# zhai-lw/L3AC

Measured on AMD Instinct MI355X. Metric: audio samples/sec encode+decode, 1kbps@16kHz, batch 256; indices bit-exact, higher is better.
Workload: dtype f32

## Files before the change

include/l3ac_hip.h:

```cpp
#ifndef L3AC_HIP_H
#define L3AC_HIP_H

#include <stddef.h>
#include <stdint.h>

#ifdef __cplusplus
extern "C" {
#endif

#define L3AC_ABI_VERSION 5
#define L3AC_MAX_STAGES 8
#define L3AC_MAX_LEVELS 8

enum {
    L3AC_OK = 0,
    L3AC_EINVAL = -1,
    L3AC_EWEIGHT = -2,
    L3AC_EHIP = -3,
    L3AC_ENOMEM = -4,
    L3AC_ECOOP = -5,
};

typedef struct l3ac_config {
    int32_t abi_version;
// ... 168 lines not shown
               double fmin, double fmax, int32_t window, int32_t hop, double threshold, double* f0, int32_t* voiced, double* aperiodicity,
               double* cmnd, int32_t* frames, void* scratch, int64_t scratch_bytes, void* stream);
int l3ac_pitch_metrics(const double* f0_ref, const int32_t* voiced_ref, const double* f0_est, const int32_t* voiced_est, int32_t batch,
                       int64_t max_frames, const int32_t* frames, double* out, int32_t* counts, void* stream);

typedef struct l3ac_pack_stream_desc {
    int32_t slot;
    int32_t held;
    int32_t take;
    int32_t count;
    int32_t keep;
} l3ac_pack_stream_desc;
typedef struct l3ac_unpack_stream_desc {
    int32_t slot;
    int32_t held;
    int32_t take;
    int32_t count;
    int32_t keep;
} l3ac_unpack_stream_desc;
int64_t l3ac_packed_bytes(int64_t n_tok, int32_t bits);
int l3ac_pack_stream(const uint32_t* state_in, uint32_t* state_out, int32_t streams, const int32_t* fresh, int64_t fresh_tokens,
                     int64_t fresh_stride, int32_t bits, const l3ac_pack_stream_desc* desc, int32_t count, uint8_t* out, int64_t out_bytes,
                     int64_t out_stride, void* stream);
int l3ac_unpack_stream(const uint32_t* state_in, uint32_t* state_out, int32_t streams, const uint8_t* fresh, int64_t fresh_bytes,
                       int64_t fresh_stride, int32_t bits, const l3ac_unpack_stream_desc* desc, int32_t count, int32_t* out, int64_t out_tokens,
                       int64_t out_stride, void* stream);

int l3ac_op_first_block(l3ac_ctx* ctx, const float* audio, int32_t batch, int32_t samples, float* y, void* stream);
int l3ac_op_first_block_at(l3ac_ctx* ctx, const float* audio, int32_t batch, int32_t samples, int64_t audio_stride, int32_t frames,
                           float* y, void* stream);
int l3ac_op_conv_unit(l3ac_ctx* ctx, const char* block, const float* x, int32_t batch, int32_t frames, float* y,
                      void* stream);
int l3ac_op_down_layer(l3ac_ctx* ctx, const char* block, const float* x, int32_t batch, int32_t frames, float* y,
                       void* stream);
int l3ac_op_conv_k3(l3ac_ctx* ctx, const char* block, const float* x, int32_t batch, int32_t frames, float* y,
                    void* stream);
int l3ac_op_enhance(l3ac_ctx* ctx, const char* block, const float* x, int32_t batch, int32_t frames, float* y,
                    void* stream);
int l3ac_op_up_layer(l3ac_ctx* ctx, const char* block, const float* x, int32_t batch, int32_t frames, float* y,
                     void* stream);
int l3ac_op_enhance_up(l3ac_ctx* ctx, const char* enhance_block, const char* up_block, const float* x, int32_t batch,
                       int32_t frames, float* y, void* stream);
int l3ac_op_last_block(l3ac_ctx* ctx, const float* x, int32_t batch, int32_t frames, float* audio, void* stream);
int l3ac_op_legacy_unit(l3ac_ctx* ctx, int32_t unit, const float* x, int32_t batch, int32_t frames, float* y, void* stream);
int l3ac_op_head(l3ac_ctx* ctx, const float* x, int32_t batch, int32_t frames, float* audio, void* stream);
int l3ac_op_local_trans(l3ac_ctx* ctx, const char* block, const float* x, int32_t batch, int32_t frames, float* y,
                        void* stream);
int l3ac_op_encoder(l3ac_ctx* ctx, const float* audio, int32_t batch, int32_t samples, float* feature, void* stream);
int l3ac_op_en_encoder(l3ac_ctx* ctx, const float* feature, int32_t batch, int32_t frames, float* tokens, void* stream);
int l3ac_op_en_decoder(l3ac_ctx* ctx, const float* tokens, int32_t batch, int32_t n_tok, float* feature, void* stream);
int l3ac_op_decoder(l3ac_ctx* ctx, const float* feature, int32_t batch, int32_t frames, float* audio, void* stream);

int l3ac_op_snake(const float* x, float* y, int64_t rows, int32_t c, const float* alpha, int32_t mode, void* stream);
int l3ac_ctx_set_head_pretanh(l3ac_ctx* ctx, int32_t enable);

typedef struct l3ac_profile_entry {
    char name[64];
    int32_t launches;
    int32_t reserved;
    double ms_total;
    double flops;
    double bytes;
} l3ac_profile_entry;
int l3ac_profile_begin(void);
int l3ac_profile_end(l3ac_profile_entry* out, int32_t cap, int32_t* n_out);

int l3ac_gemm_f32(const float* a, int64_t lda, const float* w, const float* bias, float* c, int64_t ldc,
                  int64_t m, int32_t n, int32_t k, void* stream);

void l3ac_split3_host(const float* x, int64_t n, uint16_t* planes);
int l3ac_ctx_set_gemm_split(l3ac_ctx* ctx, int32_t enable);
int l3ac_ctx_set_option(l3ac_ctx* ctx, const char* name, int32_t value);
int l3ac_ctx_get_option(const l3ac_ctx* ctx, const char* name, int32_t* out);
int32_t l3ac_ctx_get_gemm_split(const l3ac_ctx* ctx);
int64_t l3ac_gemm_split_image_bytes(int32_t n, int32_t k);
int l3ac_gemm_split_image(const float* w, int32_t n, int32_t k, void* image, void* stream);
int l3ac_gemm_split_f32(const float* a, int64_t lda, const void* image, const float* bias, float* c, int64_t ldc,
                        int64_t m, int32_t n, int32_t k, void* stream);
int l3ac_gemm_split_f32_at(const float* a, int64_t lda, const void* image, const float* bias, float* c, int64_t ldc,
                           int64_t m, int32_t n, int32_t k, int32_t w256, void* stream);

#ifdef __cplusplus
}
#endif
#endif
```

l3ac_amd/_capi.py:

```python
from __future__ import annotations

import ctypes as C
from pathlib import Path

import os

LIB_PATH = Path(os.environ.get("L3AC_LIB_PATH") or Path(__file__).resolve().parent / "libl3ac_hip.so")
ABI_VERSION = 5
MAX_STAGES = 8
MAX_LEVELS = 8


class L3acError(RuntimeError):
    pass


class Config(C.Structure):
    _fields_ = [
        ("abi_version", C.c_int32),
        ("feature_dim", C.c_int32),
        ("n_enc", C.c_int32),
        ("enc_dims", C.c_int32 * MAX_STAGES),
        ("enc_depths", C.c_int32 * MAX_STAGES),
        ("compress_rates", C.c_int32 * MAX_STAGES),
# ... 28 lines not shown
    _fields_ = [("slot", C.c_int32), ("held", C.c_int32), ("take", C.c_int32), ("count", C.c_int32), ("keep", C.c_int32)]


class UnpackStreamDesc(C.Structure):
    _fields_ = [("slot", C.c_int32), ("held", C.c_int32), ("take", C.c_int32), ("count", C.c_int32), ("keep", C.c_int32)]


class Tensor(C.Structure):
    _fields_ = [("name", C.c_char_p), ("data", C.c_void_p), ("numel", C.c_int64)]


_P, _I32, _I64 = C.c_void_p, C.c_int32, C.c_int64
SIGNATURES = {
    "l3ac_last_error": (C.c_char_p, []),
    "l3ac_abi_version": (C.c_int, []),
    "l3ac_create": (C.c_int, [C.POINTER(Config), C.POINTER(Tensor), _I32, _I32, C.POINTER(_P)]),
    "l3ac_destroy": (None, [_P]),
    "l3ac_reserve": (C.c_int, [_P, _I32, _I32]),
    "l3ac_workspace_bytes": (_I64, [_P]),
    "l3ac_grn_min_norm": (C.c_int, [_P, _I32, C.POINTER(C.c_float)]),
    "l3ac_bad_index_count": (C.c_int, [_P, _I32, C.POINTER(_I64)]),
    "l3ac_coop_timeout_count": (C.c_int, [_P, _I32, C.POINTER(_I64)]),
    "l3ac_coop_timeout_pending": (C.c_int, [_P, C.POINTER(_I64)]),
    "l3ac_coop_claimed_cus": (_I32, [_I32]),
    "l3ac_hop_length": (_I32, [_P]),
    "l3ac_encode": (C.c_int, [_P, _P, _I32, _I32, _I64, _P, _P, _P, _P]),
    "l3ac_decode": (C.c_int, [_P, _P, _P, _I32, _I32, _P, _P]),
    "l3ac_encode_ragged": (C.c_int, [_P, _P, _I32, _I32, _I64, C.POINTER(_I32), _P, _P, _P, _P]),
    "l3ac_decode_ragged": (C.c_int, [_P, _P, _P, _I32, _I32, C.POINTER(_I32), _P, _P]),
    "l3ac_fsq_forward": (C.c_int, [_P, _I64, _I32, C.POINTER(_I32), _I32, _P, _P, _P, _P, _P, _P, _P, _P, _P]),
    "l3ac_fsq_quantize_act": (C.c_int, [_P, _I64, _I32, C.POINTER(_I32), _I32, _P, _P, _P, _P, _P, _P]),
    "l3ac_fsq_decode": (C.c_int, [_P, _I64, _I32, C.POINTER(_I32), _I32, _P, _P, _P, _P]),
    "l3ac_fsq_copy_ceiling": (C.c_int, [_P, _I64, _P, _P, _P, _P]),
    "l3ac_fsq_copy_ceiling_at": (C.c_int, [_P, _I64, _P, _P, _P, _I32, _P]),
    "l3ac_vq_argmin_scratch_bytes": (_I64, [_I64, _I32, _I32]),
    "l3ac_vq_argmin": (C.c_int, [_P, _I64, _P, _I32, _I32, _P, _P, _I64, _I32, _P]),
    "l3ac_op_first_block": (C.c_int, [_P, _P, _I32, _I32, _P, _P]),
    "l3ac_op_first_block_at": (C.c_int, [_P, _P, _I32, _I32, _I64, _I32, _P, _P]),
    "l3ac_op_conv_unit": (C.c_int, [_P, C.c_char_p, _P, _I32, _I32, _P, _P]),
    "l3ac_op_down_layer": (C.c_int, [_P, C.c_char_p, _P, _I32, _I32, _P, _P]),
    "l3ac_op_conv_k3": (C.c_int, [_P, C.c_char_p, _P, _I32, _I32, _P, _P]),
    "l3ac_op_enhance": (C.c_int, [_P, C.c_char_p, _P, _I32, _I32, _P, _P]),
    "l3ac_op_up_layer": (C.c_int, [_P, C.c_char_p, _P, _I32, _I32, _P, _P]),
    "l3ac_op_enhance_up": (C.c_int, [_P, C.c_char_p, C.c_char_p, _P, _I32, _I32, _P, _P]),
    "l3ac_op_last_block": (C.c_int, [_P, _P, _I32, _I32, _P, _P]),
    "l3ac_op_legacy_unit": (C.c_int, [_P, _I32, _P, _I32, _I32, _P, _P]),
    "l3ac_op_head": (C.c_int, [_P, _P, _I32, _I32, _P, _P]),
    "l3ac_op_local_trans": (C.c_int, [_P, C.c_char_p, _P, _I32, _I32, _P, _P]),
    "l3ac_op_encoder": (C.c_int, [_P, _P, _I32, _I32, _P, _P]),
    "l3ac_op_en_encoder": (C.c_int, [_P, _P, _I32, _I32, _P, _P]),
    "l3ac_op_en_decoder": (C.c_int, [_P, _P, _I32, _I32, _P, _P]),
    "l3ac_op_decoder": (C.c_int, [_P, _P, _I32, _I32, _P, _P]),
    "l3ac_op_snake": (C.c_int, [_P, _P, _I64, _I32, _P, _I32, _P]),
    "l3ac_ctx_set_head_pretanh": (C.c_int, [_P, _I32]),
    "l3ac_gemm_f32": (C.c_int, [_P, _I64, _P, _P, _P, _I64, _I64, _I32, _I32, _P]),
    "l3ac_split3_host": (None, [_P, _I64, _P]),
    "l3ac_ctx_set_gemm_split": (C.c_int, [_P, _I32]),
    "l3ac_ctx_set_option": (C.c_int, [_P, C.c_char_p, _I32]),
    "l3ac_ctx_get_option": (C.c_int, [_P, C.c_char_p, C.POINTER(_I32)]),
    "l3ac_ctx_get_gemm_split": (_I32, [_P]),
    "l3ac_gemm_split_image_bytes": (_I64, [_I32, _I32]),
    "l3ac_gemm_split_image": (C.c_int, [_P, _I32, _I32, _P, _P]),
    "l3ac_gemm_split_f32": (C.c_int, [_P, _I64, _P, _P, _P, _I64, _I64, _I32, _I32, _P]),
    "l3ac_gemm_split_f32_at": (C.c_int, [_P, _I64, _P, _P, _P, _I64, _I64, _I32, _I32, _I32, _P]),
    "l3ac_pack_indices": (C.c_int, [_P, _I32, _I32, _I32, _P, _I32, _P]),
    "l3ac_unpack_indices": (C.c_int, [_P, _I32, _I32, _I32, _I32, _P, _P]),
    "l3ac_resample_length": (_I64, [_I32, _I32, _I64]),
    "l3ac_resample_bank": (_I64, [_I32, _I32, _P, _I64]),
    "l3ac_resample": (C.c_int, [_P, _I32, _I64, _I64, _I32, _I32, _P, _P, _I64, _P]),
    "l3ac_chunk_plan": (_I64, [C.POINTER(_I64), _I32, _I64, _I64, _I32, C.POINTER(ChunkDesc), _I64]),
    "l3ac_chunk_cut": (C.c_int, [_P, _I32, _I64, _I32, C.POINTER(ChunkDesc), _I32, _P, _I32, _I64, _P]),
    "l3ac_chunk_merge": (C.c_int, [_P, _I32, _I64, _I32, C.POINTER(ChunkDesc), _I32, _P, _I32, _I64, _I64, _P]),
    "l3ac_stream_gather": (C.c_int, [_P, _I32, _I64, _P, _I64, _I64, _I32, C.POINTER(StreamDesc), _I32, _P, _I32, _I64, _P]),
    "l3ac_stream_carry": (C.c_int, [_P, _I32, _I64, _I32, C.POINTER(StreamDesc), _I32, _P, _I32, _I64, _P]),
    "l3ac_stream_append": (C.c_int, [_P, _I64, _I64, _I32, C.POINTER(StreamDesc), _I32, _P, _I32, _I64, _P]),
    "l3ac_stream_emit": (C.c_int, [_P, _I32, _I64, _I32, C.POINTER(StreamDesc), _I32, _P, _I32, _I64, _I64, _P]),
    "l3ac_resample_stream_state": (_I64, [_I32, _I32]),
    "l3ac_resample_stream": (C.c_int, [_P, _P, _I32, _I64, _P, _I64, _I64, _I32, _I32, _P, C.POINTER(ResampleStreamDesc), _I32, _P, _I64, _I64, _P]),
    "l3ac_packed_bytes": (_I64, [_I64, _I32]),
    "l3ac_pack_stream": (C.c_int, [_P, _P, _I32, _P, _I64, _I64, _I32, C.POINTER(PackStreamDesc), _I32, _P, _I64, _I64, _P]),
    "l3ac_unpack_stream": (C.c_int, [_P, _P, _I32, _P, _I64, _I64, _I32, C.POINTER(UnpackStreamDesc), _I32, _P, _I64, _I64, _P]),
    "l3ac_stft_frames": (_I64, [_I64, _I32]),
    "l3ac_stft_basis": (_I64, [_I32, _P, _I64]),
    "l3ac_mel_weights": (_I64, [_I32, _I32, _I32, _P, _I64]),
    "l3ac_mel_scratch_bytes": (_I64, [_I32, _I64, _I32, _I32, _I32]),
    "l3ac_stft": (C.c_int, [_P, _I32, _I64, _I64, C.POINTER(_I32), _I32, _I32, _P, _P, _P, _I64, _P]),
    "l3ac_log_mel": (C.c_int, [_P, _I32, _I64, _I64, C.POINTER(_I32), _I32, _I32, _P, _P, _I32, _P, _P, _I64, _P]),
    "l3ac_mel_distance": (C.c_int, [_P, _I64, _P, _I64, _I32, _I64, C.POINTER(_I32), _I32, _I32, _I32, _P, _P, _P, _P, _I64, _P]),
    "l3ac_signal_metrics": (C.c_int, [_P, _I64, _P, _I64, _I32, _I64, C.POINTER(_I32), _P, _P, _I64, _P]),
    "l3ac_stoi_frames": (_I64, [_I64]),
    "l3ac_stoi_basis": (_I64, [_P, _I64]),
    "l3ac_stoi_window": (_I64, [_P, _I64]),
    "l3ac_stoi_bands": (C.c_int, [C.POINTER(_I32)]),
    "l3ac_stoi_scratch_bytes": (_I64, [_I32, _I64]),
    "l3ac_stoi": (C.c_int, [_P, _I64, _P, _I64, _I32, _I64, C.POINTER(_I32), _P, _P, _P, _P, _P, _I64, _P]),
    "l3ac_loudness_coeffs": (_I64, [_I32, _P, _I64]),
    "l3ac_loudness_blocks": (_I64, [_I64, _I32]),
    "l3ac_loudness_scratch_bytes": (_I64, [_I32, _I64, _I32]),
    "l3ac_loudness": (C.c_int, [_P, _I64, _I32, _I64, C.POINTER(_I32), _I32, _P, _P, _P, _P, _I64, _P]),
    "l3ac_loudness_gain": (C.c_int, [_P, _I32, C.c_double, C.c_double, _P, _P]),
    "l3ac_apply_gain": (C.c_int, [_P, _I64, _P, _I64, _I32, _I64, C.POINTER(_I32), _P, _I64, _P]),
    "l3ac_pitch_lags": (C.c_int, [_I32, C.c_double, C.c_double, _I32, _I32, C.POINTER(_I32)]),
    "l3ac_pitch_frames": (_I64, [_I64, _I32, C.c_double, C.c_double, _I32, _I32]),
    "l3ac_pitch_scratch_bytes": (_I64, [_I32, _I64, _I32, C.c_double, C.c_double, _I32, _I32]),
    "l3ac_pitch": (C.c_int, [_P, _I64, _I32, _I64, C.POINTER(_I32), _I32, C.c_double, C.c_double, _I32, _I32, C.c_double, _P, _P, _P, _P, _P, _P,
                             _I64, _P]),
# ... 164 lines not shown
```

l3ac_amd/build.py:

```python
from __future__ import annotations

import os
import shutil
import subprocess
import sys
from concurrent.futures import ThreadPoolExecutor
from pathlib import Path

PKG = Path(__file__).resolve().parent
REPO = PKG.parent
CSRC = PKG / "csrc"
_TAG = os.environ.get("L3AC_BUILD_TAG", "")
OBJ_DIR = CSRC / (f"build_{_TAG}" if _TAG else "build")
LIB_PATH = PKG / (f"libl3ac_hip_{_TAG}.so" if _TAG else "libl3ac_hip.so")
ARCH = "gfx950"

SOURCES = [
    "capi.hip",
    "network.hip",
    "kernels/gemm_f32.hip",
    "kernels/gemm_split.hip",
    "kernels/gemm_split_w256.hip",
    "kernels/rows.hip",
    "kernels/first_block.hip",
# ... 79 lines not shown
        return []
    return extra


def _flag_stamp(hipcc: str, flags) -> str:
    import hashlib
    ver = subprocess.run([hipcc, "--version"], capture_output=True, text=True).stdout
    per_file = "\n".join(f"{k}: {' '.join(_per_file_flags(hipcc, k))}" for k in sorted(PER_FILE_FLAGS))
    return hashlib.sha256(("\n".join(flags) + "\n" + per_file + "\n" + ver).encode()).hexdigest()


def build_library(force: bool = False, verbose: bool = False) -> Path:
    OBJ_DIR.mkdir(parents=True, exist_ok=True)
    hipcc = _hipcc()
    flags = [*os.environ.get("L3AC_EXTRA_HIPCC_FLAGS", "").split(), "-O3", "-std=c++17", f"--offload-arch={ARCH}", "-fPIC", "-Wall", "-Wno-unused-function",
             f"-I{REPO / 'include'}", f"-I{CSRC}"]
    hdr_time = _newest_header()
    stamp_file = OBJ_DIR / "flags.sha256"
    stamp = _flag_stamp(hipcc, flags)
    if not stamp_file.exists() or stamp_file.read_text().strip() != stamp:
        force = True
    jobs = []
    objs = []
    for src in SOURCES:
        s = CSRC / src
        o = OBJ_DIR / (src.replace("/", "_") + ".o")
        d = o.with_suffix(".d")
        objs.append(o)
        stale = force or not o.exists()
        if not stale:
            newest = max(s.stat().st_mtime, _depfile_newest(d) if d.exists() else hdr_time)
            stale = o.stat().st_mtime < newest
        if stale:
            jobs.append([hipcc, *flags, *_per_file_flags(hipcc, src), "-MD", "-MF", str(d), "-c", str(s), "-o", str(o)])

    def run(cmd):
        if verbose:
            print(" ".join(cmd), flush=True)
        r = subprocess.run(cmd, capture_output=True, text=True)
        if r.returncode != 0:
            raise RuntimeError(f"hipcc failed: {' '.join(cmd)}\n{r.stdout}\n{r.stderr}")
        if verbose and r.stderr.strip():
            print(r.stderr, file=sys.stderr)

    with ThreadPoolExecutor(max_workers=min(4, os.cpu_count() or 1)) as pool:
        list(pool.map(run, jobs))
    stamp_file.write_text(stamp + "\n")
    linked = bool(jobs) or not LIB_PATH.exists()
    if linked:
        run([hipcc, "-shared", "-fPIC", f"--offload-arch={ARCH}", "-o", str(LIB_PATH), *map(str, objs)])
    global last_build_report
    last_build_report = {"objects": len(objs), "compiled": len(jobs), "reused": len(objs) - len(jobs), "linked": linked,
                         "forced": bool(force)}
    return LIB_PATH


last_build_report = None


if __name__ == "__main__":
    path = build_library(force="--force" in sys.argv, verbose=True)
    r = last_build_report
    print(f"built {path} ({path.stat().st_size / 1e6:.1f} MB): {r['compiled']} of {r['objects']} objects compiled, {r['reused']} reused")
```

l3ac_amd/csrc/capi.hip:

```cpp
#include <algorithm>
#include <cmath>
#include <cstdarg>
#include <cstdlib>
#include <cstring>
#include <new>
#include <string>
#include <vector>

#include "network.hpp"
#include "kernels/split_bf16.hpp"

static thread_local std::string g_last_error;

void l3ac_set_error(const char* fmt, ...) {
    char buf[1024];
    va_list ap;
    va_start(ap, fmt);
    vsnprintf(buf, sizeof(buf), fmt, ap);
    va_end(ap);
    g_last_error = buf;
}

int l3ac_device_cu_count() {
    static std::atomic<int> cus[L3AC_MAX_DEVICES] = {};
    const int slot = l3ac_device_slot();
    int v = slot >= 0 ? cus[slot].load(std::memory_order_relaxed) : 0;
    if (v <= 0) {
        int dev = 0;
        if (hipGetDevice(&dev) != hipSuccess || hipDeviceGetAttribute(&v, hipDeviceAttributeMultiprocessorCount, dev) != hipSuccess || v <= 0) v = 256;
        if (slot >= 0) cus[slot].store(v, std::memory_order_relaxed);
    }
    return v;
}

static thread_local Profiler* g_profiler = nullptr;
Profiler* l3ac_current_profiler() { return g_profiler; }
void l3ac_set_current_profiler(Profiler* p) { g_profiler = p; }

namespace {

struct DeviceGuard {
    int prev = -1;
    bool ok = true;
    explicit DeviceGuard(int dev) {
        if (hipGetDevice(&prev) != hipSuccess) prev = -1;
        if (prev != dev && hipSetDevice(dev) != hipSuccess) ok = false;
        if (prev == dev) prev = -1;
    }
    ~DeviceGuard() {
        if (prev >= 0) (void)hipSetDevice(prev);
    }
};

#define L3AC_ENTER(ctx)                                     \
    L3AC_REQUIRE((ctx) != nullptr, "null context");         \
    DeviceGuard guard_((ctx)->device);                      \
    L3AC_REQUIRE(guard_.ok, "cannot select device %d", (ctx)->device)
// ... 836 lines not shown
        out[slot].launches += 1;
        out[slot].ms_total += ms;
        out[slot].flops += r.flops;
        out[slot].bytes += r.bytes;
    }
    if (p->failed && rc == L3AC_OK) {
        l3ac_set_error("profile: event creation failed");
        rc = L3AC_EHIP;
    }
    delete p;
    if (n_out) *n_out = n;
    return rc;
}

int l3ac_gemm_f32(const float* a, int64_t lda, const float* w, const float* bias, float* c, int64_t ldc, int64_t m,
                  int32_t n, int32_t k, void* stream) {
    GemmArgs g{};
    g.a = a; g.lda = lda; g.w = w; g.ldw = k; g.c = c; g.ldc = ldc; g.m = m; g.n = n; g.k = k; g.bias = bias; g.epi = EPI_BIAS;
    return launch_gemm((hipStream_t)stream, g);
}

void l3ac_split3_host(const float* x, int64_t n, uint16_t* planes) {
    for (int64_t i = 0; i < n; ++i) {
        uint16_t pl[3];
        split3_host(x[i], pl);
        planes[i] = pl[0];
        planes[n + i] = pl[1];
        planes[2 * n + i] = pl[2];
    }
}

int l3ac_ctx_set_head_pretanh(l3ac_ctx* ctx, int32_t enable) { return l3ac_ctx_set_option(ctx, "head_pretanh", enable); }

int l3ac_op_snake(const float* x, float* y, int64_t rows, int32_t c, const float* alpha, int32_t mode, void* stream) {
    L3AC_REQUIRE(x && y && alpha && rows >= 0 && c > 0 && c % 4 == 0 && c <= 4096 && mode >= 0 && mode <= 4, "op_snake: bad arguments");
    hipStream_t s = (hipStream_t)stream;
    float* inv = nullptr;
    std::vector<float> ha((size_t)c), hi((size_t)c);
    L3AC_HIP_CHECK(hipMemcpyAsync(ha.data(), alpha, (size_t)c * sizeof(float), hipMemcpyDeviceToHost, s));
    L3AC_HIP_CHECK(hipStreamSynchronize(s));
    for (int i = 0; i < c; ++i) hi[i] = 1.0f / (ha[i] + 1e-8f);
    L3AC_HIP_CHECK(hipMalloc((void**)&inv, (size_t)c * sizeof(float)));
    int rc = L3AC_OK;
    if (hipMemcpyAsync(inv, hi.data(), (size_t)c * sizeof(float), hipMemcpyHostToDevice, s) != hipSuccess) {
        l3ac_set_error("op_snake: upload failed");
        rc = L3AC_EHIP;
    }
    if (rc == L3AC_OK) rc = launch_snake(s, x, y, rows, c, alpha, inv, mode);
    (void)hipStreamSynchronize(s);
    (void)hipFree(inv);
    return rc;
}

int l3ac_ctx_set_option(l3ac_ctx* ctx, const char* name, int32_t value) {
    L3AC_REQUIRE(ctx != nullptr && name != nullptr, "set_option: null argument");
    if (std::strcmp(name, "coop_release_claim") == 0) {
        trans_coop_release(ctx->coop);
        return L3AC_OK;
    }
    if (std::strcmp(name, "coop_test_fault") == 0) {
        ctx->coop.fault_part = value - 1;
        return L3AC_OK;
    }
    const Option* o = find_option(name);
    return o ? set_checked(ctx, *o, value, "set_option") : unknown_option("set_option", name);
}

int l3ac_ctx_get_option(const l3ac_ctx* ctx, const char* name, int32_t* out) {
    L3AC_REQUIRE(ctx != nullptr && name != nullptr && out != nullptr, "get_option: null argument");
    const Option* o = find_option(name);
    if (!o) return unknown_option("get_option", name);
    *out = o->field(const_cast<l3ac_ctx&>(*ctx));
    return L3AC_OK;
}

int l3ac_ctx_set_gemm_split(l3ac_ctx* ctx, int32_t enable) { return l3ac_ctx_set_option(ctx, "gemm_split", enable); }
int32_t l3ac_ctx_get_gemm_split(const l3ac_ctx* ctx) { int32_t v = 0; return l3ac_ctx_get_option(ctx, "gemm_split", &v) == L3AC_OK ? v : 0; }

int64_t l3ac_gemm_split_image_bytes(int32_t n, int32_t k) {
    return (n > 0 && k > 0 && gemm_split_eligible(n, k)) ? gemm_split_image_bytes(n, k) : 0;
}

int l3ac_gemm_split_image(const float* w, int32_t n, int32_t k, void* image, void* stream) {
    L3AC_REQUIRE(gemm_split_eligible(n, k), "split image: shape n=%d k=%d is not eligible (n >= 192, k >= 32, k %% 8 == 0)", n, k);
    return launch_gemm_split_image((hipStream_t)stream, w, k, n, k, (unsigned char*)image);
}

int l3ac_gemm_split_f32_at(const float* a, int64_t lda, const void* image, const float* bias, float* c, int64_t ldc, int64_t m,
                           int32_t n, int32_t k, int32_t w256, void* stream) {
    L3AC_REQUIRE(w256 >= 0 && w256 <= 2, "split gemm: w256 = %d, not 0, 1 or 2", w256);
    GemmArgs g{};
    g.a = a; g.lda = lda; g.w_img = (const unsigned char*)image; g.c = c; g.ldc = ldc; g.m = m; g.n = n; g.k = k; g.bias = bias;
    g.epi = EPI_BIAS; g.w256 = w256;
    return launch_gemm_split((hipStream_t)stream, g);
}
int l3ac_gemm_split_f32(const float* a, int64_t lda, const void* image, const float* bias, float* c, int64_t ldc, int64_t m,
                        int32_t n, int32_t k, void* stream) {
    const Option& o = *find_option("gemm_w256");
    return l3ac_gemm_split_f32_at(a, lda, image, bias, c, ldc, m, n, k, checked_value(o, initial_value(o)), stream);
}

}
```

l3ac_amd/csrc/kernels/gemm_split_common.hpp:

```cpp
#pragma once

#include <type_traits>

#include "../kernels.hpp"
#include "device_math.hpp"
#include "gemm_epilogue.hpp"
#include "split_bf16.hpp"

namespace {

constexpr int BM = 128, BN = 128, BK = 32, THREADS = 256;
constexpr int W_PLANE = BN * 64;
constexpr int W_TILE = 3 * W_PLANE;
constexpr int W_LOADS = W_TILE / (16 * THREADS);
static_assert(W_TILE == L3AC_SPLIT_TILE_BYTES, "image geometry");

__host__ __device__ __forceinline__ int tile_off(int row, int chunk) { return row * 64 + ((chunk ^ ((0 - (row >> 2)) & 3)) << 4); }

typedef float f32x4a __attribute__((ext_vector_type(4)));
__device__ __forceinline__ void c_store(float* p, float v) { __builtin_nontemporal_store(v, p); }

template <int RG, int NT = 8>
__device__ __forceinline__ void gemm_epilogue16(const GemmArgs& p, f32x4a (&acc)[RG][NT], int64_t m0, int n0, int wave, int lane) {
    const int c32 = lane & 31, hi = lane >> 5;
// ... 54 lines not shown
                        f32x2 hv;
                        hv.x = half ? up[i] : lo[i];
                        hv.y = half ? up[i + 1] : lo[i + 1];
                        const f32x2 sv = snake_act2(hv + bi, al, ia);
                        const f32x2 o = p.epi == EPI_SNAKE_GRN ? __builtin_elementwise_fma(ga, sv, be) + sv : sv;
                        const int64_t m = mw + 16 * h + 4 * half + i;
                        if (m < p.m) c_store(p.c + m * p.ldc + n, o.x);
                        if (m + 1 < p.m) c_store(p.c + (m + 1) * p.ldc + n, o.y);
                    }
                continue;
            }
#pragma unroll
            for (int half = 0; half < 2; ++half)
#pragma unroll
                for (int i = 0; i < 4; ++i) {
                    const int64_t m = mw + 16 * h + 4 * half + i;
                    if (m >= p.m) continue;
                    float v = (half ? up[i] : lo[i]) + bias;
                    if (p.epi == EPI_BIAS_RES) v = p.res[m * p.ldres + n] + v;
                    c_store(p.c + m * p.ldc + n, v);
                }
        }
    }
}

template <int RG, int NQ, class AccAt>
__device__ __forceinline__ void epilogue_rows(const GemmArgs& p, AccAt&& acc_at, int64_t m0, int n0, int wave, int lane, float* tb) {
    {
    const int er = lane >> 4, eq = lane & 15, ln = lane & 15, lg = lane >> 4;
    const int64_t mw = m0 + 16 * RG * wave;
#pragma unroll
    for (int sq = 0; sq < NQ; ++sq) {
        const int col = n0 + 64 * sq + 4 * eq;
        const bool col_ok = col < p.n;
        const int colc = col_ok ? col : 0;
        typedef float f4 __attribute__((ext_vector_type(4)));
        const f4 bias = p.bias ? *reinterpret_cast<const f4*>(p.bias + colc) : f4{0.f, 0.f, 0.f, 0.f};
        f4 alpha = {0.f, 0.f, 0.f, 0.f}, inv_alpha = alpha, gamma = alpha, beta = alpha;
        if (p.epi == EPI_SNAKE || p.epi == EPI_SNAKE_GRN) {
            alpha = *reinterpret_cast<const f4*>(p.alpha + colc);
            inv_alpha = *reinterpret_cast<const f4*>(p.inv_alpha + colc);
        }
        if (p.epi == EPI_SNAKE_GRN) {
            gamma = *reinterpret_cast<const f4*>(p.gamma + colc);
            beta = *reinterpret_cast<const f4*>(p.beta + colc);
        }
#pragma unroll
        for (int h = 0; h < RG; ++h) {
            float* const sb = tb + 1024 * ((sq * RG + h) & 1);
#pragma unroll
            for (int tt = 0; tt < 4; ++tt)
#pragma unroll
                for (int i = 0; i < 4; ++i) sb[(4 * lg + i) * 64 + 16 * tt + ln] = acc_at(sq, h, tt)[i];
#pragma unroll
            for (int jr = 0; jr < 4; ++jr) {
                const int64_t m = mw + 16 * h + er + 4 * jr;
                f4 v = *reinterpret_cast<const f4*>(sb + (er + 4 * jr) * 64 + 4 * eq);
                if (m >= p.m || !col_ok) continue;
                v = v + bias;
                if (p.epi == EPI_SNAKE || p.epi == EPI_SNAKE_GRN) {
                    const f32x2 s0 = snake_act2(f32x2{v.x, v.y}, f32x2{alpha.x, alpha.y}, f32x2{inv_alpha.x, inv_alpha.y});
                    const f32x2 s1 = snake_act2(f32x2{v.z, v.w}, f32x2{alpha.z, alpha.w}, f32x2{inv_alpha.z, inv_alpha.w});
                    if (p.epi == EPI_SNAKE_GRN) {
                        const f32x2 o0 = __builtin_elementwise_fma(f32x2{gamma.x, gamma.y}, s0, f32x2{beta.x, beta.y}) + s0;
                        const f32x2 o1 = __builtin_elementwise_fma(f32x2{gamma.z, gamma.w}, s1, f32x2{beta.z, beta.w}) + s1;
                        v = f4{o0.x, o0.y, o1.x, o1.y};
                    } else {
                        v = f4{s0.x, s0.y, s1.x, s1.y};
                    }
                } else if (p.epi == EPI_BIAS_RES) {
                    v = *reinterpret_cast<const f4*>(p.res + m * p.ldres + col) + v;
                }
                __builtin_nontemporal_store(v, reinterpret_cast<f4*>(p.c + m * p.ldc + col));
            }
        }
    }
}
}

template <int N, class F, int I = 0>
__device__ __forceinline__ void tail_for(F&& f) {
    if constexpr (I < N) {
        f(std::integral_constant<int, I>{});
        tail_for<N, F, I + 1>(static_cast<F&&>(f));
    }
}

}
```

l3ac_amd/csrc/kernels/rows.hip:

```cpp
#include "../kernels.hpp"
#include "device_math.hpp"
#include "lane_sums.hpp"

namespace {

constexpr int THREADS = 256;
constexpr int MAX_CH = 2;

__device__ __forceinline__ float group_sum(float v, int lpr, int pos) {
    if ((lpr & (lpr - 1)) == 0) return lanes_sum(v, lpr);
    for (int d = 1; d < lpr; d <<= 1) {
        const float o = __shfl_down(v, d, 64);
        v += pos + d < lpr ? o : 0.f;
    }
    return __shfl(v, (int)(threadIdx.x & 63) - pos, 64);
}

__device__ __forceinline__ float4 f4_fma(float4 a, float4 b, float4 c) {
    return make_float4(fmaf(a.x, b.x, c.x), fmaf(a.y, b.y, c.y), fmaf(a.z, b.z, c.z), fmaf(a.w, b.w, c.w));
}

template <int SRC, int NORM, class IDX, int LPR, int NCH>
__global__ __launch_bounds__(THREADS) void row_kernel(const RowArgs p, const int lpr_rt) {
    const int lpr = LPR ? LPR : lpr_rt;
    const int gpw = 64 / lpr;
    const int lane = threadIdx.x & 63;
    const int grp = lane / lpr;
    const int j = lane - grp * lpr;
    const IDX rows = (IDX)(p.batch * p.frames_out);
    const IDX frames_out = (IDX)p.frames_out, frames_in = (IDX)p.frames_in, cc = (IDX)p.c;
    const int nchunk = p.c >> 2;
    const IDX wave_id = (IDX)blockIdx.x * (THREADS / 64) + (threadIdx.x >> 6);
    const IDX row_step = (IDX)gridDim.x * (THREADS / 64) * gpw;
    for (IDX row = grp < gpw ? wave_id * gpw + grp : rows; row < rows; row += row_step) {
    const bool row_ok = true;
    const IDX b = row / frames_out;
    const IDX t = row - b * frames_out;

    float4 v[NCH];
    bool ok[NCH];
#pragma unroll
    for (int i = 0; i < NCH; ++i) {
        const int chunk = j + i * lpr;
        ok[i] = row_ok && chunk < nchunk;
        v[i] = make_float4(0.f, 0.f, 0.f, 0.f);
        if (!ok[i]) continue;
        const int c0 = chunk << 2;
        if (SRC == SRC_PLAIN) {
            v[i] = *reinterpret_cast<const float4*>(p.x + (size_t)((b * frames_in + t) * cc + (IDX)c0));
        } else if (SRC == SRC_DWCONV7) {
            float4 acc = *reinterpret_cast<const float4*>(p.dw_b + c0);
#pragma unroll
            for (int tap = 0; tap < 7; ++tap) {
                const int64_t ts = (int64_t)t + tap - 3;
                if (ts >= 0 && ts < p.frames_in) {
                    const float4 xv = *reinterpret_cast<const float4*>(p.x + (size_t)((b * frames_in + (IDX)ts) * cc + (IDX)c0));
                    const float4 wv = *reinterpret_cast<const float4*>(p.dw_w + tap * p.c + c0);
                    acc = f4_fma(xv, wv, acc);
                }
            }
// ... 26 lines not shown
            const float4 xv = *reinterpret_cast<const float4*>(p.x + (size_t)((b * frames_in + t) * cc + (IDX)c0));
            const float4 gb = *reinterpret_cast<const float4*>(p.gate_b + c0);
            const float xs[4] = {xv.x, xv.y, xv.z, xv.w};
            const float gbs[4] = {gb.x, gb.y, gb.z, gb.w};
            float o[4];
#pragma unroll
            for (int e = 0; e < 4; ++e) {
                const float4 gw = *reinterpret_cast<const float4*>(p.gate_w + (int64_t)(c0 + e) * 4);
                const float g = gbs[e] + gw.x * y0 + gw.y * y1 + gw.z * y2 + gw.w * y3;
                o[e] = xs[e] + g * xs[e];
            }
            v[i] = make_float4(o[0], o[1], o[2], o[3]);
        }
    }

    if (NORM != NORM_NONE) {
        float s = 0.f;
#pragma unroll
        for (int i = 0; i < NCH; ++i) s += (v[i].x + v[i].y) + (v[i].z + v[i].w);
        const float mean = group_sum(s, lpr, j) / (float)p.c;
        float q = 0.f;
#pragma unroll
        for (int i = 0; i < NCH; ++i) {
            if (ok[i]) {
                const float dx = v[i].x - mean, dy = v[i].y - mean, dz = v[i].z - mean, dw = v[i].w - mean;
                q += (dx * dx + dy * dy) + (dz * dz + dw * dw);
            }
        }
        const float var = group_sum(q, lpr, j) / (float)p.c;
        const float rstd = 1.0f / sqrtf(var + p.eps);
#pragma unroll
        for (int i = 0; i < NCH; ++i) {
            if (!ok[i]) continue;
            const int c0 = (j + i * lpr) << 2;
            const float4 w = *reinterpret_cast<const float4*>(p.nw + c0);
            const float4 bb = *reinterpret_cast<const float4*>(p.nb + c0);
            if (NORM == NORM_LN) {
                v[i] = make_float4((v[i].x - mean) * rstd * w.x + bb.x, (v[i].y - mean) * rstd * w.y + bb.y,
                                   (v[i].z - mean) * rstd * w.z + bb.z, (v[i].w - mean) * rstd * w.w + bb.w);
            } else {
                v[i] = make_float4(w.x * ((v[i].x - mean) * rstd) + bb.x, w.y * ((v[i].y - mean) * rstd) + bb.y,
                                   w.z * ((v[i].z - mean) * rstd) + bb.z, w.w * ((v[i].w - mean) * rstd) + bb.w);
            }
        }
    }
#pragma unroll
    for (int i = 0; i < NCH; ++i) {
        if (ok[i]) *reinterpret_cast<float4*>(p.y + (size_t)(row * cc + (IDX)((j + i * lpr) << 2))) = v[i];
    }
    }
}


template <int CH>
__global__ __launch_bounds__(THREADS) void dwconv_ln_kernel(const RowArgs p, const int lpr, const int DW_SEG) {
    const int groups_per_block = THREADS / lpr;
    const int64_t seg_per_clip = (p.frames_out + DW_SEG - 1) / DW_SEG;
    const int64_t seg = (int64_t)blockIdx.x * groups_per_block + threadIdx.x / lpr;
    const int j = threadIdx.x % lpr;
    const bool seg_ok = seg < p.batch * seg_per_clip;
    const int64_t sg = seg_ok ? seg : 0;
    const int64_t b = sg / seg_per_clip;
    const int t0 = (int)(sg % seg_per_clip) * DW_SEG;
    const int frames = (int)p.frames_in;
    const int nchunk = p.c >> 2;
    const float* clip = p.x + b * p.frames_in * p.c;
    float* dst = p.y + b * p.frames_in * p.c;

    bool ok[CH];
    int c0[CH];
    float4 wt[7][CH], bias[CH], lw[CH], lb[CH], win[7][CH];
#pragma unroll
    for (int i = 0; i < CH; ++i) {
        const int chunk = j + i * lpr;
        ok[i] = seg_ok && chunk < nchunk;
        c0[i] = (ok[i] ? chunk : 0) << 2;
        bias[i] = *reinterpret_cast<const float4*>(p.dw_b + c0[i]);
        lw[i] = *reinterpret_cast<const float4*>(p.nw + c0[i]);
        lb[i] = *reinterpret_cast<const float4*>(p.nb + c0[i]);
#pragma unroll
        for (int tap = 0; tap < 7; ++tap) wt[tap][i] = *reinterpret_cast<const float4*>(p.dw_w + tap * p.c + c0[i]);
    }
    auto load_row = [&](int t, int i) -> float4 {
        if (ok[i] && t >= 0 && t < frames) return *reinterpret_cast<const float4*>(clip + (int64_t)t * p.c + c0[i]);
        return make_float4(0.f, 0.f, 0.f, 0.f);
    };
#pragma unroll
    for (int d = -3; d <= 2; ++d)
#pragma unroll
        for (int i = 0; i < CH; ++i) win[(d + 7) % 7][i] = load_row(t0 + d, i);

    for (int base = 0; base < DW_SEG; base += 7) {
#pragma unroll
        for (int u = 0; u < 7; ++u) {
            const int t = t0 + base + u;
#pragma unroll
            for (int i = 0; i < CH; ++i) win[(u + 3) % 7][i] = load_row(t + 3, i);
            float4 v[CH];
            float s = 0.f;
#pragma unroll
            for (int i = 0; i < CH; ++i) {
                float4 acc = bias[i];
#pragma unroll
                for (int tap = 0; tap < 7; ++tap) acc = f4_fma(win[(u + tap + 4) % 7][i], wt[tap][i], acc);
                v[i] = ok[i] ? acc : make_float4(0.f, 0.f, 0.f, 0.f);
                s += (v[i].x + v[i].y) + (v[i].z + v[i].w);
            }
            const float mean = group_sum(s, lpr, j) / (float)p.c;
            float q = 0.f;
#pragma unroll
            for (int i = 0; i < CH; ++i) {
                if (ok[i]) {
                    const float dx = v[i].x - mean, dy = v[i].y - mean, dz = v[i].z - mean, dw = v[i].w - mean;
                    q += (dx * dx + dy * dy) + (dz * dz + dw * dw);
                }
            }
            const float rstd = 1.0f / sqrtf(group_sum(q, lpr, j) / (float)p.c + p.eps);
            if (t < frames) {
#pragma unroll
                for (int i = 0; i < CH; ++i) {
                    if (!ok[i]) continue;
                    *reinterpret_cast<float4*>(dst + (int64_t)t * p.c + c0[i]) =
                        make_float4((v[i].x - mean) * rstd * lw[i].x + lb[i].x, (v[i].y - mean) * rstd * lw[i].y + lb[i].y,
                                    (v[i].z - mean) * rstd * lw[i].z + lb[i].z, (v[i].w - mean) * rstd * lw[i].w + lb[i].w);
                }
            }
        }
    }
}

int launch_dwconv_ln(hipStream_t s, const RowArgs& r, int lpr) {
    const int64_t rows_per_wave_group = (r.batch * r.frames_out * lpr / 64) / (256 * 4 * 6);
    int DW_SEG = (int)(rows_per_wave_group / 7) * 7;
    DW_SEG = DW_SEG < 7 ? 7 : (DW_SEG > 56 ? 56 : DW_SEG);
    const int64_t segs = r.batch * ((r.frames_out + DW_SEG - 1) / DW_SEG);
    const int64_t blocks = ceil_div64(segs, THREADS / lpr);
    if (blocks <= 0) return L3AC_OK;
    L3AC_REQUIRE(blocks < (int64_t)1 << 31, "rows: grid too large");
    const double elems = (double)r.batch * r.frames_out * r.c;
    ProfScope prof(s, "dwconv_ln_kernel", 22.0 * elems, 8.0 * elems);
    if (r.c <= 4 * lpr)
        hipLaunchKernelGGL((dwconv_ln_kernel<1>), dim3((unsigned)blocks), dim3(THREADS), 0, s, r, lpr, DW_SEG);
    else
        hipLaunchKernelGGL((dwconv_ln_kernel<2>), dim3((unsigned)blocks), dim3(THREADS), 0, s, r, lpr, DW_SEG);
    L3AC_LAUNCH_CHECK();
    return L3AC_OK;
}

template <int SRC, int NORM>
int launch_rows_t(hipStream_t s, const RowArgs& r, int lpr) {
    const int64_t rows = r.batch * r.frames_out;
    int64_t blocks = ceil_div64(rows, (THREADS / 64) * (64 / lpr));
    if (blocks <= 0) return L3AC_OK;
    if (SRC == SRC_LERP && blocks > 256 * 32) blocks = 256 * 32;
    static const char* const names[4][3] = {{"row_kernel<PLAIN,NONE>", "row_kernel<PLAIN,LN>", "row_kernel<PLAIN,CN>"},
                                            {"row_kernel<DWCONV7,NONE>", "row_kernel<DWCONV7,LN>", "row_kernel<DWCONV7,CN>"},
                                            {"row_kernel<LERP,NONE>", "row_kernel<LERP,LN>", "row_kernel<LERP,CN>"},
                                            {"row_kernel<GATE,NONE>", "row_kernel<GATE,LN>", "row_kernel<GATE,CN>"}};
    const double in_elems = (double)r.batch * r.frames_in * r.c, out_elems = (double)rows * r.c;
    ProfScope prof(s, names[SRC][NORM], (SRC == SRC_DWCONV7 ? 14.0 : 2.0) * out_elems + (NORM != NORM_NONE ? 8.0 * out_elems : 0.0),
                   4.0 * (in_elems + out_elems));
    const bool small = (double)r.batch * r.frames_in * r.c < 2147483648.0 && out_elems < 2147483648.0 && rows + blocks * 256 < ((int64_t)1 << 31);
#define L3AC_ROWS_LAUNCH(IDX_, LPR_)                                                                                             \
    do {                                                                                                                         \
        if (r.c <= 4 * lpr)                                                                                                      \
            hipLaunchKernelGGL((row_kernel<SRC, NORM, IDX_, LPR_, 1>), dim3((unsigned)blocks), dim3(THREADS), 0, s, r, lpr);     \
        else                                                                                                                     \
            hipLaunchKernelGGL((row_kernel<SRC, NORM, IDX_, LPR_, MAX_CH>), dim3((unsigned)blocks), dim3(THREADS), 0, s, r, lpr); \
    } while (0)
    if (!small) {
        L3AC_ROWS_LAUNCH(int64_t, 0);
    } else {
        switch (lpr) {
            case 6: L3AC_ROWS_LAUNCH(unsigned, 6); break;
            case 12: L3AC_ROWS_LAUNCH(unsigned, 12); break;
            case 32: L3AC_ROWS_LAUNCH(unsigned, 32); break;
            case 48: L3AC_ROWS_LAUNCH(unsigned, 48); break;
            case 64: L3AC_ROWS_LAUNCH(unsigned, 64); break;
            default: L3AC_ROWS_LAUNCH(unsigned, 0); break;
        }
    }
#undef L3AC_ROWS_LAUNCH
    L3AC_LAUNCH_CHECK();
    return L3AC_OK;
}

__global__ __launch_bounds__(THREADS) void snake_kernel(const float* __restrict__ x, float* __restrict__ y,
                                                       int64_t n4, int c4, const float* __restrict__ alpha,
                                                       const float* __restrict__ inv_alpha, const int mode) {
    for (int64_t i = (int64_t)blockIdx.x * THREADS + threadIdx.x; i < n4; i += (int64_t)gridDim.x * THREADS) {
        const int c0 = (int)(i % c4) << 2;
        const float4 v = reinterpret_cast<const float4*>(x)[i];
        float4 o;
        if (mode == 4) {
            o = make_float4(gelu_erf(v.x), gelu_erf(v.y), gelu_erf(v.z), gelu_erf(v.w));
        } else if (mode & 2) {
            if (mode & 1) {
// ... 177 lines not shown
```

Measured before the change: 316.0 million.

## Prefetch rows ahead in dwconv+LN kernel and retune segment length

```diff
diff --git a/include/l3ac_hip.h b/include/l3ac_hip.h
--- a/include/l3ac_hip.h
+++ b/include/l3ac_hip.h
@@ -244,6 +244,8 @@
 int l3ac_op_decoder(l3ac_ctx* ctx, const float* feature, int32_t batch, int32_t frames, float* audio, void* stream);
 
 int l3ac_op_snake(const float* x, float* y, int64_t rows, int32_t c, const float* alpha, int32_t mode, void* stream);
+int l3ac_op_dwconv_ln(const float* x, float* y, int32_t batch, int32_t frames, int32_t c, const float* dw_w, const float* dw_b,
+                      const float* ln_w, const float* ln_b, void* stream);
 int l3ac_ctx_set_head_pretanh(l3ac_ctx* ctx, int32_t enable);
 
 typedef struct l3ac_profile_entry {
diff --git a/l3ac_amd/_capi.py b/l3ac_amd/_capi.py
--- a/l3ac_amd/_capi.py
+++ b/l3ac_amd/_capi.py
@@ -104,6 +104,7 @@
     "l3ac_op_en_decoder": (C.c_int, [_P, _P, _I32, _I32, _P, _P]),
     "l3ac_op_decoder": (C.c_int, [_P, _P, _I32, _I32, _P, _P]),
     "l3ac_op_snake": (C.c_int, [_P, _P, _I64, _I32, _P, _I32, _P]),
+    "l3ac_op_dwconv_ln": (C.c_int, [_P, _P, _I32, _I32, _I32, _P, _P, _P, _P, _P]),
     "l3ac_ctx_set_head_pretanh": (C.c_int, [_P, _I32]),
     "l3ac_gemm_f32": (C.c_int, [_P, _I64, _P, _P, _P, _I64, _I64, _I32, _I32, _P]),
     "l3ac_split3_host": (None, [_P, _I64, _P]),
diff --git a/l3ac_amd/build.py b/l3ac_amd/build.py
--- a/l3ac_amd/build.py
+++ b/l3ac_amd/build.py
@@ -155,7 +155,23 @@
     global last_build_report
     last_build_report = {"objects": len(objs), "compiled": len(jobs), "reused": len(objs) - len(jobs), "linked": linked,
                          "forced": bool(force)}
+    if not _TAG:
+        _build_test_kernels(hipcc, force, run)
     return LIB_PATH
+
+
+TEST_KERNEL_DIR = REPO / "tests" / "native"
+TEST_KERNEL_LIB = TEST_KERNEL_DIR / "libl3ac_test_kernels.so"
+
+
+def _build_test_kernels(hipcc: str, force: bool, run) -> None:
+    srcs = sorted(TEST_KERNEL_DIR.glob("*.hip"))
+    if not srcs:
+        return
+    newest = max(max(f.stat().st_mtime for f in srcs), (CSRC / "kernels" / "lane_sums.hpp").stat().st_mtime)
+    if force or not TEST_KERNEL_LIB.exists() or TEST_KERNEL_LIB.stat().st_mtime < newest:
+        run([hipcc, "-O3", "-std=c++17", f"--offload-arch={ARCH}", "-fPIC", "-shared", "-Wall", "-Wno-unused-function", f"-I{CSRC}",
+             "-o", str(TEST_KERNEL_LIB), *map(str, srcs)])
 
 
 last_build_report = None
diff --git a/l3ac_amd/csrc/capi.hip b/l3ac_amd/csrc/capi.hip
--- a/l3ac_amd/csrc/capi.hip
+++ b/l3ac_amd/csrc/capi.hip
@@ -3,6 +3,7 @@
 #include <cstdarg>
 #include <cstdlib>
 #include <cstring>
+#include <initializer_list>
 #include <new>
 #include <string>
 #include <vector>
@@ -945,6 +946,21 @@
     return rc;
 }
 
+int l3ac_op_dwconv_ln(const float* x, float* y, int32_t batch, int32_t frames, int32_t c, const float* dw_w, const float* dw_b,
+                      const float* ln_w, const float* ln_b, void* stream) {
+    L3AC_REQUIRE(x && y && x != y && dw_w && dw_b && ln_w && ln_b && batch > 0 && frames > 0 && c > 0 && c % 4 == 0 && c <= 512,
+                 "op_dwconv_ln: bad arguments");
+    for (const void* q : {(const void*)x, (const void*)y, (const void*)dw_w, (const void*)dw_b, (const void*)ln_w, (const void*)ln_b})
+        L3AC_REQUIRE(((uintptr_t)q & 15) == 0, "op_dwconv_ln: pointers must be 16-byte aligned");
+    hipStream_t s = (hipStream_t)stream;
+    RowArgs r{};
+    r.x = x; r.y = y; r.batch = batch; r.frames_in = frames; r.frames_out = frames; r.c = c;
+    r.src = SRC_DWCONV7; r.norm = NORM_LN; r.dw_w = dw_w; r.dw_b = dw_b; r.nw = ln_w; r.nb = ln_b; r.eps = 1e-8f;
+    L3AC_TRY(launch_rows(s, r));
+    L3AC_HIP_CHECK(hipStreamSynchronize(s));
+    return L3AC_OK;
+}
+
 int l3ac_ctx_set_option(l3ac_ctx* ctx, const char* name, int32_t value) {
     L3AC_REQUIRE(ctx != nullptr && name != nullptr, "set_option: null argument");
     if (std::strcmp(name, "coop_release_claim") == 0) {
diff --git a/l3ac_amd/csrc/kernels/gemm_split_common.hpp b/l3ac_amd/csrc/kernels/gemm_split_common.hpp
--- a/l3ac_amd/csrc/kernels/gemm_split_common.hpp
+++ b/l3ac_amd/csrc/kernels/gemm_split_common.hpp
@@ -130,6 +130,9 @@
             for (int tt = 0; tt < 4; ++tt)
 #pragma unroll
                 for (int i = 0; i < 4; ++i) sb[(4 * lg + i) * 64 + 16 * tt + ln] = acc_at(sq, h, tt)[i];
+            __builtin_amdgcn_fence(__ATOMIC_RELEASE, "wavefront");
+            __builtin_amdgcn_wave_barrier();
+            __builtin_amdgcn_fence(__ATOMIC_ACQUIRE, "wavefront");
 #pragma unroll
             for (int jr = 0; jr < 4; ++jr) {
                 const int64_t m = mw + 16 * h + er + 4 * jr;
@@ -151,6 +154,8 @@
                 }
                 __builtin_nontemporal_store(v, reinterpret_cast<f4*>(p.c + m * p.ldc + col));
             }
+            __builtin_amdgcn_fence(__ATOMIC_RELEASE, "wavefront");
+            __builtin_amdgcn_wave_barrier();
         }
     }
 }
diff --git a/l3ac_amd/csrc/kernels/rows.hip b/l3ac_amd/csrc/kernels/rows.hip
--- a/l3ac_amd/csrc/kernels/rows.hip
+++ b/l3ac_amd/csrc/kernels/rows.hip
@@ -6,6 +6,7 @@
 
 constexpr int THREADS = 256;
 constexpr int MAX_CH = 2;
+constexpr int DW_AHEAD = 4;
 
 __device__ __forceinline__ float group_sum(float v, int lpr, int pos) {
     if ((lpr & (lpr - 1)) == 0) return lanes_sum(v, lpr);
@@ -138,8 +139,9 @@
 }
 
 
-template <int CH>
-__global__ __launch_bounds__(THREADS) void dwconv_ln_kernel(const RowArgs p, const int lpr, const int DW_SEG) {
+template <int CH, int LPR, int PF>
+__global__ __launch_bounds__(THREADS, PF ? 2 : 1) void dwconv_ln_kernel(const RowArgs p, const int lpr_rt, const int DW_SEG) {
+    const int lpr = LPR ? LPR : lpr_rt;
     const int groups_per_block = THREADS / lpr;
     const int64_t seg_per_clip = (p.frames_out + DW_SEG - 1) / DW_SEG;
     const int64_t seg = (int64_t)blockIdx.x * groups_per_block + threadIdx.x / lpr;
@@ -168,6 +170,11 @@
         for (int tap = 0; tap < 7; ++tap) wt[tap][i] = *reinterpret_cast<const float4*>(p.dw_w + tap * p.c + c0[i]);
     }
     auto load_row = [&](int t, int i) -> float4 {
+        if (PF) {
+            const int tc = t < 0 ? 0 : (t < frames ? t : frames - 1);
+            const float4 v = *reinterpret_cast<const float4*>(clip + (int64_t)tc * p.c + c0[i]);
+            return ok[i] && tc == t ? v : make_float4(0.f, 0.f, 0.f, 0.f);
+        }
         if (ok[i] && t >= 0 && t < frames) return *reinterpret_cast<const float4*>(clip + (int64_t)t * p.c + c0[i]);
         return make_float4(0.f, 0.f, 0.f, 0.f);
     };
@@ -175,13 +182,27 @@
     for (int d = -3; d <= 2; ++d)
 #pragma unroll
         for (int i = 0; i < CH; ++i) win[(d + 7) % 7][i] = load_row(t0 + d, i);
+    float4 ahead[PF ? PF : 1][CH];
+#pragma unroll
+    for (int d = 0; d < PF; ++d)
+#pragma unroll
+        for (int i = 0; i < CH; ++i) ahead[d][i] = load_row(t0 + 3 + d, i);
 
     for (int base = 0; base < DW_SEG; base += 7) {
 #pragma unroll
         for (int u = 0; u < 7; ++u) {
             const int t = t0 + base + u;
 #pragma unroll
-            for (int i = 0; i < CH; ++i) win[(u + 3) % 7][i] = load_row(t + 3, i);
+            for (int i = 0; i < CH; ++i) {
+                if (PF) {
+                    win[(u + 3) % 7][i] = ahead[0][i];
+#pragma unroll
+                    for (int d = 0; d + 1 < PF; ++d) ahead[d][i] = ahead[d + 1][i];
+                    ahead[PF ? PF - 1 : 0][i] = load_row(t + 3 + PF, i);
+                } else {
+                    win[(u + 3) % 7][i] = load_row(t + 3, i);
+                }
+            }
             float4 v[CH];
             float s = 0.f;
 #pragma unroll
@@ -219,6 +240,9 @@
     const int64_t rows_per_wave_group = (r.batch * r.frames_out * lpr / 64) / (256 * 4 * 6);
     int DW_SEG = (int)(rows_per_wave_group / 7) * 7;
     DW_SEG = DW_SEG < 7 ? 7 : (DW_SEG > 56 ? 56 : DW_SEG);
+    const bool ahead = r.c > 4 * lpr;
+    if (ahead)
+        for (DW_SEG = 7; DW_SEG < 56 && r.batch * ((r.frames_out + DW_SEG - 1) / DW_SEG) > 256 * 8; DW_SEG += 7) {}
     const int64_t segs = r.batch * ((r.frames_out + DW_SEG - 1) / DW_SEG);
     const int64_t blocks = ceil_div64(segs, THREADS / lpr);
     if (blocks <= 0) return L3AC_OK;
@@ -226,9 +250,9 @@
     const double elems = (double)r.batch * r.frames_out * r.c;
     ProfScope prof(s, "dwconv_ln_kernel", 22.0 * elems, 8.0 * elems);
     if (r.c <= 4 * lpr)
-        hipLaunchKernelGGL((dwconv_ln_kernel<1>), dim3((unsigned)blocks), dim3(THREADS), 0, s, r, lpr, DW_SEG);
+        hipLaunchKernelGGL((dwconv_ln_kernel<1, 0, 0>), dim3((unsigned)blocks), dim3(THREADS), 0, s, r, lpr, DW_SEG);
     else
-        hipLaunchKernelGGL((dwconv_ln_kernel<2>), dim3((unsigned)blocks), dim3(THREADS), 0, s, r, lpr, DW_SEG);
+        hipLaunchKernelGGL((dwconv_ln_kernel<2, 64, DW_AHEAD>), dim3((unsigned)blocks), dim3(THREADS), 0, s, r, lpr, DW_SEG);
     L3AC_LAUNCH_CHECK();
     return L3AC_OK;
 }
```

Result: no change. 316.5 million (median of 2 runs) (+0.2%).
